# eigenkernel/eigenkernel

Measured on AMD Instinct MI355X. Metric: eigenpairs/s (full spectrum) + achieved fp64 TFLOP/s vs roofline, N=16384 GEP, higher is better.
Workload: dtype f64

## Files before the change

eigenkernel_amd/csrc/ek_common.h:

```cpp
#pragma once
#include <hip/hip_runtime.h>
#include <cstddef>
#include <cstdint>
#include <cstdio>

#define EK_HIP_CHECK(expr)                                                              \
  do {                                                                                  \
    hipError_t _e = (expr);                                                             \
    if (_e != hipSuccess) {                                                             \
      fprintf(stderr, "[ek_hip] %s failed at %s:%d: %s\n", #expr, __FILE__, __LINE__,   \
              hipGetErrorString(_e));                                                   \
      return -1000 - (int)_e;                                                           \
    }                                                                                   \
  } while (0)

namespace ek {

constexpr int kWave = 64;

inline int ceil_div(int a, int b) { return (a + b - 1) / b; }
inline int round_up(int a, int b) { return ceil_div(a, b) * b; }

struct GemmDesc {
  int M, N, K;
  bool transA, transB;
  double alpha, beta;
  const double *A; int lda; long long strideA;
  const double *B; int ldb; long long strideB;
  double *C; int ldc; long long strideC;
  int batch;
  bool lower_only;
  bool staged_rank_k = false;
  const long long *d_offs = nullptr;
  const int *d_dims = nullptr;
  bool even_offs = false;
  bool small_tiles = false;
};
void gemm(hipStream_t s, const GemmDesc &g);

enum { kGemmNone = -1, kGemmSmall = 0, kGemmW4 = 1, kGemmW8 = 2, kGemmRankK = 3 };
struct GemmPlan {
  int kernel;
  bool vec;
  int lower_only;
  int tile;
  int tiles_m, tiles_n;
  unsigned grid_x;
};
GemmPlan gemm_plan(const GemmDesc &g);
bool gemm_compact_tile(int tiles_m, int tiles_n, int tile, int &tm, int &tn);

inline void gemm(hipStream_t s, bool ta, bool tb, int M, int N, int K, double alpha,
                 const double *A, int lda, const double *B, int ldb, double beta, double *C,
                 int ldc, bool lower_only = false, bool staged_rank_k = false, bool small_tiles = false) {
  GemmDesc g{M, N, K, ta, tb, alpha, beta, A, lda, 0, B, ldb, 0, C, ldc, 0, 1, lower_only, staged_rank_k};
  g.small_tiles = small_tiles;
  gemm(s, g);
}

enum { kProfQ2Apply = 0, kProfChase = 1, kProfSymm = 2, kProfSyr2k = 3, kProfCount = 4 };
void kprof_enable(bool on);
bool kprof_enabled();
void kprof_begin(hipStream_t s, int id);
void kprof_end(hipStream_t s, int id);
void kprof_collect(double *seconds , long long *launches );

void copy_matrix(hipStream_t s, int m, int n, const double *src, int lds, double *dst, int ldd);
void set_matrix(hipStream_t s, int m, int n, double offdiag, double diag, double *A, int lda);
void symmetrize_lower(hipStream_t s, int n, double *A, int lda);
void transpose_rows(hipStream_t s, int n, int m, const double *src, int lds, int r0, double *dst, int ldd);
void gather_columns(hipStream_t s, int m, int n, const double *src, int lds, const int *perm,
                    double *dst, int ldd);

void gather_block_cyclic(hipStream_t s, int mr, int nc, const double *src, int lds, int nb, int pr,
                         int me_r, int pc, int me_c, double *dst, int ldd);

void scatter_block_cyclic(hipStream_t s, int mr, int nc, const double *src, int lds, int nb, int pr,
                          int me_r, int pc, int me_c, double *dst, int ldd);

void maxabs_lower(hipStream_t s, int n, const double *A, int lda, double *partial , int bw = 1 << 30);
void scale_lower(hipStream_t s, int n, double alpha, double *A, int lda);
void scale_vector(hipStream_t s, int n, double alpha, double *x);

// ... 140 lines not shown
```

eigenkernel_amd/csrc/ek_debug.hip:

```cpp
#include "ek_api_internal.h"

using namespace ek;
using namespace ek::api;

extern "C" {

int ek_hip_potrf_team(int n, double *B_loc, const int desc_B[9], int nteam, long long *mismatch) {
  if (n < 0) return -1;
  if (!B_loc && n > 0) return -2;
  int rc = check_desc(desc_B, 3, n, n); if (rc) return rc;
  if (nteam < 0 || nteam > kMaxTeam) return -4;
  rc = ensure_init(); if (rc) return rc;
  if (mismatch) *mismatch = 0;
  if (n == 0) return 0;
  std::lock_guard<std::mutex> lk(g_mu);
  if (nteam == 0 && !g_comm.on) return -4;
  hipStream_t s = g_ctx.stream;
  const int ld = pad_ld(n), nblk = ceil_div(n, kDiagNB);
  const int nmem = nteam > 0 ? nteam : 1, P = nteam > 0 ? nteam : g_comm.nranks;
  const size_t wb = potrf_dist_work_bytes(n, ld, P);
  const size_t per = al((size_t)ld * ld * 8) + al((size_t)nblk * kDiagNB * kDiagNB * 8) + al(wb) + 256;
  void *ws;
  rc = workspace(per * nmem + 256, &ws);
  if (rc) return rc;
// ... 695 lines not shown
  DevMem mem;
  if (offs && batch > 0) {
    double *p; rc = mem.alloc(&p, (size_t)3 * batch * sizeof(long long)); if (rc) return rc;
    EK_HIP_CHECK(hipMemcpy(p, offs, (size_t)3 * batch * sizeof(long long), hipMemcpyHostToDevice));
    g.d_offs = reinterpret_cast<const long long *>(p);
  }
  if (dims && batch > 0) {
    double *p; rc = mem.alloc(&p, (size_t)3 * batch * sizeof(int)); if (rc) return rc;
    EK_HIP_CHECK(hipMemcpy(p, dims, (size_t)3 * batch * sizeof(int), hipMemcpyHostToDevice));
    g.d_dims = reinterpret_cast<const int *>(p);
  }
  gemm_variant_out(gemm_plan(g), batch, variant);
  gemm(s, g);
  EK_HIP_CHECK(hipGetLastError());
  EK_HIP_CHECK(hipStreamSynchronize(s));
  return 0;
}

int ek_hip_debug_gemm_compact_map(int tiles_m, int tiles_n, long long first, int count, int *tm, int *tn, int *valid) {
  if (tiles_m < 1) return -1;
  if (tiles_n < 1 || tiles_n > tiles_m) return -2;
  if (first < 0) return -3;
  if (count < 0 || first + count > 0x7fffffffLL) return -4;
  if (count > 0 && (!tm || !tn)) return -5;
  int ok = 0;
  for (int i = 0; i < count; ++i) {
    const bool v = gemm_compact_tile(tiles_m, tiles_n, (int)(first + i), tm[i], tn[i]);
    if (valid) valid[i] = v ? 1 : 0;
    ok += v ? 1 : 0;
  }
  return ok;
}

int ek_hip_debug_sytrd_split(void *alt, int mask) {
  std::lock_guard<std::mutex> lk(g_mu);
  sytrd_debug_split(alt, mask);
  return 0;
}

int ek_hip_debug_set_sytrd_maxcols(int max_cols) {
  std::lock_guard<std::mutex> lk(g_mu);
  sytrd_set_max_cols(max_cols);
  return 0;
}

}
```

eigenkernel_amd/csrc/ek_gemm.hip:

```cpp
#include "ek_common.h"

#include <cmath>
#include <cstdlib>

namespace ek {
namespace {

typedef double double4_t __attribute__((ext_vector_type(4)));

constexpr int BM = 128, BN = 128, BK = 16;
constexpr int MC_LD = BM + 16;
constexpr int KC_LD = BK + 1;
constexpr int TILE_DOUBLES = (BK * MC_LD > BM * KC_LD) ? BK * MC_LD : BM * KC_LD;

struct GemmArgs {
  int M, N, K;
  double alpha, beta;
  const double *A; int lda; long long sA;
  const double *B; int ldb; long long sB;
  double *C; int ldc; long long sC;
  int lower_only;
  int tiles_m, tiles_n;
  const long long *offs;
  const int *dims;
};

template <bool KCONTIG>
__device__ __forceinline__ void load_slab(double (&r)[8], const double *__restrict__ P, int ld,
                                          int x0, int X, int k0, int K, int t) {
#pragma unroll
  for (int i = 0; i < 8; ++i) {
    const int idx = t + 256 * i;
    int x, k;
    if (KCONTIG) { k = idx & 15; x = idx >> 4; }
    else         { x = idx & 127; k = idx >> 7; }
    const int gx = x0 + x, gk = k0 + k;
    double v = 0.0;
    if (gx < X && gk < K)
      v = KCONTIG ? P[(size_t)gk + (size_t)gx * ld] : P[(size_t)gx + (size_t)gk * ld];
    r[i] = v;
  }
}

template <bool KCONTIG>
__device__ __forceinline__ void store_slab(const double (&r)[8], double *s, int t) {
// ... 8 lines not shown
typedef double double2g_t __attribute__((ext_vector_type(2)));
template <bool KCONTIG>
__device__ __forceinline__ void load_slab_v(double (&r)[8], const double *__restrict__ P, int ld, int x0, int X,
                                            int k0, int K, int t) {
  if (x0 + BM <= X && k0 + BK <= K) {
#pragma unroll
    for (int i = 0; i < 4; ++i) {
      const int idx = t + 256 * i;
      double2g_t v;
      if (KCONTIG) v = *reinterpret_cast<const double2g_t *>(P + (size_t)(k0 + 2 * (idx & 7)) + (size_t)(x0 + (idx >> 3)) * ld);
      else         v = *reinterpret_cast<const double2g_t *>(P + (size_t)(x0 + 2 * (idx & 63)) + (size_t)(k0 + (idx >> 6)) * ld);
      r[2 * i] = v.x; r[2 * i + 1] = v.y;
    }
  } else {
#pragma unroll
    for (int i = 0; i < 4; ++i) {
      const int idx = t + 256 * i;
#pragma unroll
      for (int h = 0; h < 2; ++h) {
        const int gx = x0 + (KCONTIG ? (idx >> 3) : 2 * (idx & 63) + h);
        const int gk = k0 + (KCONTIG ? 2 * (idx & 7) + h : (idx >> 6));
        double v = 0.0;
        if (gx < X && gk < K) v = KCONTIG ? P[(size_t)gk + (size_t)gx * ld] : P[(size_t)gx + (size_t)gk * ld];
        r[2 * i + h] = v;
      }
    }
  }
}
template <bool KCONTIG>
__device__ __forceinline__ void store_slab_v(const double (&r)[8], double *s, int t) {
#pragma unroll
  for (int i = 0; i < 4; ++i) {
    const int idx = t + 256 * i;
    if (KCONTIG) { const int k = 2 * (idx & 7), x = idx >> 3; s[x * KC_LD + k] = r[2 * i]; s[x * KC_LD + k + 1] = r[2 * i + 1]; }
    else { const int x = 2 * (idx & 63), k = idx >> 6; *reinterpret_cast<double2g_t *>(&s[k * MC_LD + x]) = (double2g_t){r[2 * i], r[2 * i + 1]}; }
  }
}

template <bool KCONTIG>
__device__ __forceinline__ double frag(const double *s, int x, int k) {
  return KCONTIG ? s[x * KC_LD + k] : s[k * MC_LD + x];
}

__host__ __device__ __forceinline__ bool tile_of(const GemmArgs &p, int tile, int &tm, int &tn) {
  if (p.lower_only == 2) {
    const long long T = p.tiles_m, c = tile;
    int j = (int)(((double)(2 * T + 1) - sqrt((double)((2 * T + 1) * (2 * T + 1) - 8 * c))) * 0.5);
    if (j < 0) j = 0;
    if (j > p.tiles_n - 1) j = p.tiles_n - 1;
    while (j + 1 < p.tiles_n && (long long)(j + 1) * T - (long long)(j + 1) * j / 2 <= c) ++j;
    while (j > 0 && (long long)j * T - (long long)j * (j - 1) / 2 > c) --j;
    tn = j; tm = j + (int)(c - ((long long)j * T - (long long)j * (j - 1) / 2));
    return tm < p.tiles_m;
  }
  tm = tile % p.tiles_m; tn = tile / p.tiles_m;
  return true;
}

template <bool TA, bool TB, bool VEC>
__global__ __launch_bounds__(256, 2) void gemm_kernel(GemmArgs p) {
  __shared__ __attribute__((aligned(16))) double smem[2 * TILE_DOUBLES];
  double *sA = smem, *sB = smem + TILE_DOUBLES;

  int tm, tn;
  if (!tile_of(p, blockIdx.x, tm, tn)) return;
  const int m0 = tm * BM, n0 = tn * BN;
  if (p.lower_only && n0 > m0 + BM - 1) return;
  if (p.dims) {
    p.M = p.dims[3 * blockIdx.y]; p.N = p.dims[3 * blockIdx.y + 1]; p.K = p.dims[3 * blockIdx.y + 2];
    if (m0 >= p.M || n0 >= p.N) return;
  }

  const double *__restrict__ A = p.A + (size_t)blockIdx.y * p.sA;
  const double *__restrict__ B = p.B + (size_t)blockIdx.y * p.sB;
  double *__restrict__ C = p.C + (size_t)blockIdx.y * p.sC;
  if (p.offs) {
    A += p.offs[3 * blockIdx.y]; B += p.offs[3 * blockIdx.y + 1]; C += p.offs[3 * blockIdx.y + 2];
  }

  const int t = threadIdx.x, lane = t & 63, wave = t >> 6;
  const int wm = (wave & 1) * 64, wn = (wave >> 1) * 64;
  const int l15 = lane & 15, l4 = lane >> 4;

  double4_t acc[4][4];
#pragma unroll
  for (int i = 0; i < 4; ++i)
#pragma unroll
    for (int j = 0; j < 4; ++j) acc[i][j] = (double4_t){0.0, 0.0, 0.0, 0.0};

  double ra[8], rb[8];
  if (VEC) {
    load_slab_v<TA>(ra, A, p.lda, m0, p.M, 0, p.K, t);
    load_slab_v<!TB>(rb, B, p.ldb, n0, p.N, 0, p.K, t);
  } else {
    load_slab<TA>(ra, A, p.lda, m0, p.M, 0, p.K, t);
    load_slab<!TB>(rb, B, p.ldb, n0, p.N, 0, p.K, t);
  }

  for (int k0 = 0; k0 < p.K; k0 += BK) {
    __syncthreads();
    if (VEC) { store_slab_v<TA>(ra, sA, t); store_slab_v<!TB>(rb, sB, t); }
    else { store_slab<TA>(ra, sA, t); store_slab<!TB>(rb, sB, t); }
    __syncthreads();
    if (k0 + BK < p.K) {
      if (VEC) {
        load_slab_v<TA>(ra, A, p.lda, m0, p.M, k0 + BK, p.K, t);
        load_slab_v<!TB>(rb, B, p.ldb, n0, p.N, k0 + BK, p.K, t);
      } else {
        load_slab<TA>(ra, A, p.lda, m0, p.M, k0 + BK, p.K, t);
        load_slab<!TB>(rb, B, p.ldb, n0, p.N, k0 + BK, p.K, t);
      }
    }
#pragma unroll
    for (int kk = 0; kk < BK; kk += 4) {
      double fa[4], fb[4];
#pragma unroll
      for (int i = 0; i < 4; ++i) {
        fa[i] = frag<TA>(sA, wm + i * 16 + l15, kk + l4);
        fb[i] = frag<!TB>(sB, wn + i * 16 + l15, kk + l4);
      }
#pragma unroll
      for (int ni = 0; ni < 4; ++ni)
#pragma unroll
        for (int mi = 0; mi < 4; ++mi)
          acc[ni][mi] = __builtin_amdgcn_mfma_f64_16x16x4f64(fb[ni], fa[mi], acc[ni][mi], 0, 0, 0);
    }
  }

  const double alpha = p.alpha, beta = p.beta;
#pragma unroll
  for (int ni = 0; ni < 4; ++ni)
#pragma unroll
    for (int mi = 0; mi < 4; ++mi) {
      const int m = m0 + wm + mi * 16 + l15;
#pragma unroll
      for (int r = 0; r < 4; ++r) {
        const int n = n0 + wn + ni * 16 + l4 + 4 * r;
        if (m < p.M && n < p.N) {
          double *c = C + (size_t)m + (size_t)n * p.ldc;
          double v = alpha * acc[ni][mi][r];
          if (beta != 0.0) v += beta * *c;
          *c = v;
        }
      }
    }
}


template <bool KCONTIG>
__device__ __forceinline__ void load_slab8(double (&r)[4], const double *__restrict__ P, int ld,
                                           int x0, int X, int k0, int K, int t) {
#pragma unroll
  for (int i = 0; i < 4; ++i) {
    const int idx = t + 512 * i;
    int x, k;
    if (KCONTIG) { k = idx & 15; x = idx >> 4; }
    else         { x = idx & 127; k = idx >> 7; }
    const int gx = x0 + x, gk = k0 + k;
    double v = 0.0;
// ... 14 lines not shown

template <bool KCONTIG>
__device__ __forceinline__ void load_slab8_v(double (&r)[4], const double *__restrict__ P, int ld, int x0, int X,
                                             int k0, int K, int t) {
  if (x0 + BM <= X && k0 + BK <= K) {
#pragma unroll
    for (int i = 0; i < 2; ++i) {
      const int idx = t + 512 * i;
      double2g_t v;
      if (KCONTIG) v = *reinterpret_cast<const double2g_t *>(P + (size_t)(k0 + 2 * (idx & 7)) + (size_t)(x0 + (idx >> 3)) * ld);
      else         v = *reinterpret_cast<const double2g_t *>(P + (size_t)(x0 + 2 * (idx & 63)) + (size_t)(k0 + (idx >> 6)) * ld);
      r[2 * i] = v.x; r[2 * i + 1] = v.y;
    }
  } else {
#pragma unroll
    for (int i = 0; i < 2; ++i) {
      const int idx = t + 512 * i;
#pragma unroll
      for (int h = 0; h < 2; ++h) {
        const int gx = x0 + (KCONTIG ? (idx >> 3) : 2 * (idx & 63) + h);
        const int gk = k0 + (KCONTIG ? 2 * (idx & 7) + h : (idx >> 6));
        double v = 0.0;
        if (gx < X && gk < K) v = KCONTIG ? P[(size_t)gk + (size_t)gx * ld] : P[(size_t)gx + (size_t)gk * ld];
        r[2 * i + h] = v;
      }
    }
  }
}
template <bool KCONTIG>
__device__ __forceinline__ void store_slab8_v(const double (&r)[4], double *s, int t) {
#pragma unroll
  for (int i = 0; i < 2; ++i) {
    const int idx = t + 512 * i;
    if (KCONTIG) { const int k = 2 * (idx & 7), x = idx >> 3; s[x * KC_LD + k] = r[2 * i]; s[x * KC_LD + k + 1] = r[2 * i + 1]; }
    else { const int x = 2 * (idx & 63), k = idx >> 6; *reinterpret_cast<double2g_t *>(&s[k * MC_LD + x]) = (double2g_t){r[2 * i], r[2 * i + 1]}; }
  }
}

template <bool TA, bool TB, bool VEC>
__global__ __launch_bounds__(512, 4) void gemm_kernel_w8(GemmArgs p) {
  __shared__ __attribute__((aligned(16))) double smem[2 * TILE_DOUBLES];
  double *sA = smem, *sB = smem + TILE_DOUBLES;
  int tm, tn;
  if (!tile_of(p, blockIdx.x, tm, tn)) return;
  const int m0 = tm * BM, n0 = tn * BN;
  if (p.lower_only && n0 > m0 + BM - 1) return;
  if (p.dims) {
    p.M = p.dims[3 * blockIdx.y]; p.N = p.dims[3 * blockIdx.y + 1]; p.K = p.dims[3 * blockIdx.y + 2];
    if (m0 >= p.M || n0 >= p.N) return;
  }
  const double *__restrict__ A = p.A + (size_t)blockIdx.y * p.sA;
  const double *__restrict__ B = p.B + (size_t)blockIdx.y * p.sB;
  double *__restrict__ C = p.C + (size_t)blockIdx.y * p.sC;
  if (p.offs) {
    A += p.offs[3 * blockIdx.y]; B += p.offs[3 * blockIdx.y + 1]; C += p.offs[3 * blockIdx.y + 2];
  }
  const int t = threadIdx.x, lane = t & 63, wave = t >> 6;
  const int wm = (wave & 1) * 64, wn = (wave >> 1) * 32;
  const int l15 = lane & 15, l4 = lane >> 4;
  double4_t acc[2][4];
#pragma unroll
  for (int i = 0; i < 2; ++i)
#pragma unroll
    for (int j = 0; j < 4; ++j) acc[i][j] = (double4_t){0.0, 0.0, 0.0, 0.0};
  double ra0[4], rb0[4];
  if (VEC) {
    load_slab8_v<TA>(ra0, A, p.lda, m0, p.M, 0, p.K, t);
    load_slab8_v<!TB>(rb0, B, p.ldb, n0, p.N, 0, p.K, t);
  } else {
    load_slab8<TA>(ra0, A, p.lda, m0, p.M, 0, p.K, t);
    load_slab8<!TB>(rb0, B, p.ldb, n0, p.N, 0, p.K, t);
  }
  for (int k0 = 0; k0 < p.K; k0 += BK) {
    __syncthreads();
    if (VEC) { store_slab8_v<TA>(ra0, sA, t); store_slab8_v<!TB>(rb0, sB, t); }
    else { store_slab8<TA>(ra0, sA, t); store_slab8<!TB>(rb0, sB, t); }
    __syncthreads();
// ... 160 lines not shown
      for (int ni = 0; ni < 2; ++ni)
#pragma unroll
        for (int mi = 0; mi < 2; ++mi)
          acc[ni][mi] = __builtin_amdgcn_mfma_f64_16x16x4f64(fb[ni], fa[mi], acc[ni][mi], 0, 0, 0);
    }
  }
  const double alpha = p.alpha, beta = p.beta;
#pragma unroll
  for (int ni = 0; ni < 2; ++ni)
#pragma unroll
    for (int mi = 0; mi < 2; ++mi) {
      const int m = m0 + wm + mi * 16 + l15;
#pragma unroll
      for (int r = 0; r < 4; ++r) {
        const int n = n0 + wn + ni * 16 + l4 + 4 * r;
        if (m < p.M && n < p.N) {
          double *c = C + (size_t)m + (size_t)n * p.ldc;
          double v = alpha * acc[ni][mi][r];
          if (beta != 0.0) v += beta * *c;
          *c = v;
        }
      }
    }
}

constexpr int RK = 32;
constexpr int RK_LD = BM + 16;
typedef double double2_t __attribute__((ext_vector_type(2)));

__global__ __launch_bounds__(512) void gemm_rankk_kernel(GemmArgs p) {
  extern __shared__ double rk_smem[];
  double *sA = rk_smem, *sB = rk_smem + RK * RK_LD;
  int tm, tn;
  if (!tile_of(p, blockIdx.x, tm, tn)) return;
  const int m0 = tm * BM, n0 = tn * BN;
  if (p.lower_only && n0 > m0 + BM - 1) return;
  if (p.dims) {
    p.M = p.dims[3 * blockIdx.y]; p.N = p.dims[3 * blockIdx.y + 1]; p.K = p.dims[3 * blockIdx.y + 2];
    if (m0 >= p.M || n0 >= p.N) return;
  }
  const double *__restrict__ A = p.A + (size_t)blockIdx.y * p.sA;
  const double *__restrict__ B = p.B + (size_t)blockIdx.y * p.sB;
  double *__restrict__ C = p.C + (size_t)blockIdx.y * p.sC;
  if (p.offs) { A += p.offs[3 * blockIdx.y]; B += p.offs[3 * blockIdx.y + 1]; C += p.offs[3 * blockIdx.y + 2]; }
  const int t = threadIdx.x, lane = t & 63, wave = t >> 6;
  const int wm = (wave & 1) * 64, wn = (wave >> 1) * 32;
  const int l15 = lane & 15, l4 = lane >> 4;
  const bool vec = ((p.lda | p.ldb) & 1) == 0 && ((((size_t)A | (size_t)B) & 15) == 0);
  const int xp = 2 * (t & 63), kq = t >> 6;
  constexpr int NF = RK / 8;
  double2_t ra[NF], rb[NF];
  auto fetch = [&](int k0) {
#pragma unroll
    for (int i = 0; i < NF; ++i) {
      const int k = k0 + kq + 8 * i;
      double2_t va = (double2_t){0.0, 0.0}, vb = (double2_t){0.0, 0.0};
      if (k < p.K) {
        const double *pa = A + (size_t)(m0 + xp) + (size_t)k * p.lda;
        const double *pb = B + (size_t)(n0 + xp) + (size_t)k * p.ldb;
        if (vec && m0 + xp + 1 < p.M) va = *reinterpret_cast<const double2_t *>(pa);
        else { if (m0 + xp < p.M) va.x = pa[0]; if (m0 + xp + 1 < p.M) va.y = pa[1]; }
        if (vec && n0 + xp + 1 < p.N) vb = *reinterpret_cast<const double2_t *>(pb);
        else { if (n0 + xp < p.N) vb.x = pb[0]; if (n0 + xp + 1 < p.N) vb.y = pb[1]; }
      }
      ra[i] = va; rb[i] = vb;
    }
  };
// ... 63 lines not shown
    }
}

}

GemmPlan gemm_plan(const GemmDesc &g) {
  GemmPlan pl;
  pl.kernel = kGemmNone; pl.vec = false; pl.lower_only = 0; pl.tile = 0; pl.tiles_m = pl.tiles_n = 0; pl.grid_x = 0;
  if (g.M <= 0 || g.N <= 0 || g.batch <= 0) return pl;
  pl.lower_only = g.lower_only ? 1 : 0;
  const long long big_tiles = (long long)ceil_div(g.M, BM) * ceil_div(g.N, BN) * g.batch;
  const bool compact = g.lower_only && g.batch == 1 && !g.d_dims && !g.d_offs;
  static int vec_env = -1;
  if (vec_env < 0) { const char *e = getenv("EK_GEMM_VEC"); vec_env = e ? atoi(e) : 1; }
  pl.vec = vec_env && (!g.d_offs || g.even_offs) && ((g.lda | g.ldb) & 1) == 0 &&
           ((((size_t)g.A | (size_t)g.B) & 15) == 0) && (g.batch == 1 || ((g.strideA | g.strideB) & 1) == 0);
  const bool small = (big_tiles < 256 && !g.lower_only) || (g.lower_only && g.small_tiles);
  pl.tile = small ? SM : BM;
  pl.tiles_m = ceil_div(g.M, pl.tile); pl.tiles_n = ceil_div(g.N, pl.tile);
  pl.grid_x = (unsigned)(pl.tiles_m * pl.tiles_n);
  if (compact && pl.tiles_n <= pl.tiles_m) {
    pl.lower_only = 2;
    pl.grid_x = (unsigned)((long long)pl.tiles_n * pl.tiles_m - (long long)pl.tiles_n * (pl.tiles_n - 1) / 2);
  }
  if (small) { pl.kernel = kGemmSmall; return pl; }
  static int w8 = -2;
  if (w8 == -2) { const char *e = getenv("EK_GEMM_W8"); w8 = e ? atoi(e) : -1; }
  static int rankk = -1;
  if (rankk < 0) { const char *e = getenv("EK_GEMM_RANKK"); rankk = e ? atoi(e) : 1; }
  if (rankk && g.staged_rank_k && !g.transA && g.transB && g.K <= 256 && g.K >= 32 && w8 < 0) { pl.kernel = kGemmRankK; return pl; }
  const bool use_w8 = (w8 >= 0) ? (w8 != 0) : (g.K <= 512 && g.beta != 0.0);
  pl.kernel = use_w8 ? kGemmW8 : kGemmW4;
  return pl;
}

bool gemm_compact_tile(int tiles_m, int tiles_n, int tile, int &tm, int &tn) {
  GemmArgs p;
  p.lower_only = 2; p.tiles_m = tiles_m; p.tiles_n = tiles_n;
  return tile_of(p, tile, tm, tn);
}

void gemm(hipStream_t s, const GemmDesc &g) {
  const GemmPlan pl = gemm_plan(g);
  if (pl.kernel == kGemmNone) return;
  GemmArgs p;
  p.M = g.M; p.N = g.N; p.K = g.K > 0 ? g.K : 0;
  p.alpha = g.alpha; p.beta = g.beta;
  p.A = g.A; p.lda = g.lda; p.sA = g.strideA;
  p.B = g.B; p.ldb = g.ldb; p.sB = g.strideB;
  p.C = g.C; p.ldc = g.ldc; p.sC = g.strideC;
  p.lower_only = pl.lower_only;
  p.offs = g.d_offs; p.dims = g.d_dims;
  p.tiles_m = pl.tiles_m; p.tiles_n = pl.tiles_n;
  const bool vec = pl.vec;
  if (pl.kernel == kGemmSmall) {
    dim3 sgrid(pl.grid_x, g.batch), sblock(256);
    if (vec) {
      if (!g.transA && !g.transB) hipLaunchKernelGGL((gemm_small_kernel<false, false, true>), sgrid, sblock, 0, s, p);
      else if (!g.transA && g.transB) hipLaunchKernelGGL((gemm_small_kernel<false, true, true>), sgrid, sblock, 0, s, p);
      else if (g.transA && !g.transB) hipLaunchKernelGGL((gemm_small_kernel<true, false, true>), sgrid, sblock, 0, s, p);
      else hipLaunchKernelGGL((gemm_small_kernel<true, true, true>), sgrid, sblock, 0, s, p);
      return;
    }
    if (!g.transA && !g.transB) hipLaunchKernelGGL((gemm_small_kernel<false, false, false>), sgrid, sblock, 0, s, p);
    else if (!g.transA && g.transB) hipLaunchKernelGGL((gemm_small_kernel<false, true, false>), sgrid, sblock, 0, s, p);
    else if (g.transA && !g.transB) hipLaunchKernelGGL((gemm_small_kernel<true, false, false>), sgrid, sblock, 0, s, p);
    else hipLaunchKernelGGL((gemm_small_kernel<true, true, false>), sgrid, sblock, 0, s, p);
    return;
  }
  dim3 grid(pl.grid_x, g.batch), block(256);
  static bool rk_attr = false;
  if (!rk_attr) {
    rk_attr = true;
    (void)hipFuncSetAttribute((const void *)gemm_rankk_kernel, hipFuncAttributeMaxDynamicSharedMemorySize,
                              2 * RK * RK_LD * (int)sizeof(double));
  }
  if (pl.kernel == kGemmRankK) {
    hipLaunchKernelGGL(gemm_rankk_kernel, grid, dim3(512), 2 * RK * RK_LD * sizeof(double), s, p);
    return;
  }
  if (pl.kernel == kGemmW8) {
    dim3 b8(512);
    if (vec) {
      if (!g.transA && !g.transB) hipLaunchKernelGGL((gemm_kernel_w8<false, false, true>), grid, b8, 0, s, p);
      else if (!g.transA && g.transB) hipLaunchKernelGGL((gemm_kernel_w8<false, true, true>), grid, b8, 0, s, p);
      else if (g.transA && !g.transB) hipLaunchKernelGGL((gemm_kernel_w8<true, false, true>), grid, b8, 0, s, p);
      else hipLaunchKernelGGL((gemm_kernel_w8<true, true, true>), grid, b8, 0, s, p);
      return;
    }
    if (!g.transA && !g.transB) hipLaunchKernelGGL((gemm_kernel_w8<false, false, false>), grid, b8, 0, s, p);
    else if (!g.transA && g.transB) hipLaunchKernelGGL((gemm_kernel_w8<false, true, false>), grid, b8, 0, s, p);
    else if (g.transA && !g.transB) hipLaunchKernelGGL((gemm_kernel_w8<true, false, false>), grid, b8, 0, s, p);
    else hipLaunchKernelGGL((gemm_kernel_w8<true, true, false>), grid, b8, 0, s, p);
    return;
  }
  if (vec) {
    if (!g.transA && !g.transB) hipLaunchKernelGGL((gemm_kernel<false, false, true>), grid, block, 0, s, p);
    else if (!g.transA && g.transB) hipLaunchKernelGGL((gemm_kernel<false, true, true>), grid, block, 0, s, p);
    else if (g.transA && !g.transB) hipLaunchKernelGGL((gemm_kernel<true, false, true>), grid, block, 0, s, p);
    else hipLaunchKernelGGL((gemm_kernel<true, true, true>), grid, block, 0, s, p);
    return;
  }
  if (!g.transA && !g.transB) hipLaunchKernelGGL((gemm_kernel<false, false, false>), grid, block, 0, s, p);
  else if (!g.transA && g.transB) hipLaunchKernelGGL((gemm_kernel<false, true, false>), grid, block, 0, s, p);
  else if (g.transA && !g.transB) hipLaunchKernelGGL((gemm_kernel<true, false, false>), grid, block, 0, s, p);
  else hipLaunchKernelGGL((gemm_kernel<true, true, false>), grid, block, 0, s, p);
}

}
```

eigenkernel_amd/solver.py:

```python
import ctypes
import os
from dataclasses import dataclass, field

import numpy as np

from . import descriptor as _d

_HERE = os.path.dirname(os.path.abspath(__file__))
LIB_PATH = os.environ.get("EK_HIP_LIB") or os.path.join(_HERE, "csrc", "libek_hip.so")

N_STAGES = 8
SOLVERS = ("hip", "hip_select", "general_hip", "general_hip_select")
REPLACES = {"hip": "scalapack", "hip_select": "scalapack_select",
            "general_hip": "general_scalapack", "general_hip_select": "general_scalapack_select"}


class LibraryMissing(RuntimeError):
    pass


_lib = None
_dp = ctypes.POINTER(ctypes.c_double)
_ip = ctypes.POINTER(ctypes.c_int)
_llp = ctypes.POINTER(ctypes.c_longlong)
# ... 41 lines not shown
        "ek_hip_comm_size": (c_int, []),
        "ek_hip_comm_rank": (c_int, []),
        "ek_hip_comm_destroy": (c_int, []),
        "ek_hip_comm_allreduce_device": (c_int, [vp, ctypes.c_longlong]),
        "ek_hip_stedc": (c_int, [c_int, _dp, _dp, _dp, _ip]),
        "ek_hip_ormtr": (c_int, [c_int, c_int, _dp, _ip, _dp, _dp, _ip]),
        "ek_hip_trtrs": (c_int, [c_int, c_int, _dp, _ip, _dp, _ip]),
        "ek_hip_dgemm": (c_int, [c_int, c_int, c_int, c_int, c_int, c_dbl, _dp, c_int, _dp, c_int,
                                 c_dbl, _dp, c_int, c_int]),
        "ek_hip_malloc": (c_int, [ctypes.POINTER(vp), c_ull]),
        "ek_hip_free": (c_int, [vp]),
        "ek_hip_memcpy_h2d": (c_int, [vp, vp, c_ull]),
        "ek_hip_memcpy_d2h": (c_int, [vp, vp, c_ull]),
        "ek_hip_synchronize": (c_int, []),
        "ek_hip_synth_matrix_device": (c_int, [c_int, c_ull, vp, c_int]),
        "ek_hip_residual_device": (c_int, [c_int, c_int, c_int, vp, c_int, vp, c_int, vp, vp, c_int, _dp, _dp, _dp]),
        "ek_hip_orthogonality_device": (c_int, [c_int, c_int, c_int, c_int, vp, c_int, vp, c_int, _dp]),
        "ek_hip_ipratios_device": (c_int, [c_int, c_int, c_int, vp, c_int, vp, c_int, _dp]),
        "ek_hip_check": (c_int, [c_int, c_int, c_int, c_int, c_int, c_int, _dp, _ip, _dp, _ip, _dp, _dp, _ip, _dp]),
        "ek_hip_profile_symv": (c_int, [c_int]),
        "ek_hip_debug_sytrd": (c_int, [c_int, c_int, c_int, _dp]),
        "ek_hip_debug_sytrd_team": (c_int, [c_int, c_int, c_int, _dp]),
        "ek_hip_debug_set_sytrd_maxcols": (c_int, [c_int]),
        "ek_hip_debug_sytrd_work_bytes": (ctypes.c_ulonglong, [c_int]),
        "ek_hip_debug_sytrd_split": (c_int, [vp, c_int]),
        "ek_hip_debug_gemm_at": (c_int, [c_int, c_int, c_int, c_int, c_int, vp, c_int, vp, c_int, c_dbl, vp, c_int,
                                         c_int, c_int, _dp]),
        "ek_hip_debug_sytrd_at": (c_int, [c_int, c_int, c_int, vp, vp, vp, _dp]),
        "ek_hip_debug_gemm_desc": (c_int, [c_int] * 5 + [c_dbl, c_dbl, vp, c_int, c_ll, vp, c_int, c_ll, vp, c_int, c_ll]
                                   + [c_int] * 5 + [_llp, _ip, _ip]),
        "ek_hip_debug_gemm_plan": (c_int, [c_int] * 5 + [c_dbl, c_dbl, vp, c_int, c_ll, vp, c_int, c_ll, vp, c_int, c_ll]
                                   + [c_int] * 5 + [_llp, _ip, _ip]),
        "ek_hip_debug_gemm_compact_map": (c_int, [c_int, c_int, c_ll, c_int, _ip, _ip, _ip]),
        "ek_hip_debug_reduce_team": (c_int, [c_int, c_int, c_int, _dp]),
        "ek_hip_profile_symv_get": (c_int, [_dp, ctypes.POINTER(ctypes.c_longlong), _dp]),
        "ek_hip_debug_sy2sb": (c_int, [c_int, _dp, c_int, _dp, c_int, _dp, _ip]),
        "ek_hip_debug_sb2st": (c_int, [c_int, _dp, c_int, _dp, _dp, _dp, c_int, c_int, _ip]),
        "ek_hip_debug_two_stage_timing": (c_int, [c_int, c_int, c_int, _dp, _ip]),
        "ek_hip_debug_set_two_stage": (c_int, [c_int]),
        "ek_hip_profile_kernels": (c_int, [c_int]),
        "ek_hip_profile_kernels_get": (c_int, [_dp, _llp]),
        "ek_hip_debug_last_solve_stats": (c_int, [_dp, c_int]),
        "ek_hip_debug_sy2sb_team": (c_int, [c_int, _dp, c_int, _dp, c_int, _dp, c_int, _ip, _llp]),
        "ek_hip_debug_sy2sb_team_timing": (c_int, [c_int, c_int, c_int, _dp]),
        "ek_hip_debug_sy2sb_team_profile": (c_int, [c_int, c_int, c_int, c_int, _dp, _dp]),
        "ek_hip_debug_fail_next_chase": (c_int, [c_int]),
        "ek_hip_debug_stedc_team": (c_int, [c_int, c_int, c_int]),
        "ek_hip_debug_potrf_team_profile": (c_int, [c_int, c_int]),
        "ek_hip_debug_potrf_team_profile_get": (c_int, [c_int, _dp]),
        "ek_hip_debug_stedc_team_get": (c_int, [_dp]),
        "ek_hip_debug_last_pipe_stats": (c_int, [_dp, c_int]),
        "ek_hip_debug_workspace_bytes": (ctypes.c_ulonglong, [c_int, c_int, c_int, c_int, ctypes.POINTER(ctypes.c_ulonglong)]),
        "ek_hip_eigenvalues_device": (c_int, [c_int, c_int, c_int, c_int, vp, c_int, vp, c_int, vp, _dp, c_int]),
        "ek_hip_eigenvalues": (c_int, [c_int, c_int, c_int, c_int, _dp, c_int, _dp, c_int, _dp, _dp, c_int]),
        "ek_hip_stebz": (c_int, [c_int, _dp, _dp, c_int, c_int, _dp]),
        "ek_hip_debug_values_workspace_bytes": (ctypes.c_ulonglong, [c_int, c_int]),
        "ek_hip_debug_set_stebz": (c_int, [c_int]),
        "ek_hip_eigenpairs_device": (c_int, [c_int, c_int, c_int, c_int, c_dbl, c_dbl, c_int, c_int, vp, c_int, vp, c_int,
                                             _ip, _ip, vp, vp, c_int, c_int, _dp, c_int]),
        "ek_hip_eigenpairs": (c_int, [c_int, c_int, c_int, c_int, c_dbl, c_dbl, c_int, c_int, _dp, c_int, _dp, c_int,
                                      _ip, _ip, _dp, _dp, c_int, c_int, _dp, c_int]),
        "ek_hip_stebz_range": (c_int, [c_int, _dp, _dp, c_dbl, c_dbl, _ip, _ip, _dp]),
        "ek_hip_debug_window_workspace_bytes": (ctypes.c_ulonglong, [c_int, c_int, c_int, c_int, c_int]),
        "ek_hip_sygvx_device": (c_int, [c_int, c_int, c_int, c_int, c_dbl, c_dbl, c_int, c_int, vp, c_int, vp, c_int,
                                        _ip, _ip, vp, vp, c_int, c_int, _dp, c_int]),
        "ek_hip_sygvx": (c_int, [c_int, c_int, c_int, c_int, c_dbl, c_dbl, c_int, c_int, _dp, c_int, _dp, c_int,
# ... 19 lines not shown
        "ek_hip_check_batched": (c_int, [c_int, c_int, c_int, _dp, c_int, c_ll, _dp, c_int, c_ll, _dp, _dp, c_int, c_ll,
                                         _ip, _dp, _dp, _dp]),
        "ek_hip_check_vbatched_device": (c_int, [c_int, c_int, _ip, vp, _ip, vp, _ip, vp, vp, _ip, _ip, _dp, vp, _dp]),
        "ek_hip_check_vbatched": (c_int, [c_int, c_int, _ip, vp, _ip, vp, _ip, vp, vp, _ip, _ip, _dp, vp, _dp]),
        "ek_hip_debug_vbatched_streams": (c_int, [c_int]),
        "ek_hip_debug_vbatched_last": (c_int, [_dp, _ip]),
    }
    for name, (res, args) in sigs.items():
        try:
            fn = getattr(lib, name)
        except AttributeError:
            if os.environ.get("EK_HIP_BRINGUP") == "1":
                continue
            raise
        fn.restype = res
        fn.argtypes = args
    if path is None:
        _lib = lib
    return lib


EXPORTED_SYMBOLS = (
    "ek_hip_version", "ek_hip_init", "ek_hip_finalize", "ek_hip_stage_name", "ek_hip_solve",
    "ek_hip_solve_device", "ek_hip_solve_replicated", "ek_hip_solve_device_grid",
    "ek_hip_set_allgatherv", "ek_hip_gather_matrix", "ek_hip_potrf", "ek_hip_sygst", "ek_hip_sytrd", "ek_hip_stedc",
    "ek_hip_ormtr", "ek_hip_trtrs", "ek_hip_dgemm", "ek_hip_malloc", "ek_hip_free",
    "ek_hip_memcpy_h2d", "ek_hip_memcpy_d2h", "ek_hip_synchronize", "ek_hip_synth_matrix_device",
    "ek_hip_profile_symv", "ek_hip_profile_symv_get", "ek_hip_debug_sytrd",
    "ek_hip_residual_device", "ek_hip_orthogonality_device", "ek_hip_ipratios_device", "ek_hip_check",
    "ek_hip_sytrd_team", "ek_hip_comm_unique_id", "ek_hip_comm_init", "ek_hip_comm_size", "ek_hip_comm_rank",
    "ek_hip_comm_destroy", "ek_hip_comm_allreduce_device", "ek_hip_debug_sytrd_team", "ek_hip_sygst_team",
    "ek_hip_potrf_team", "ek_hip_debug_reduce_team", "ek_hip_comm_attach_host",
    "ek_hip_debug_set_sytrd_maxcols", "ek_hip_debug_sytrd_work_bytes", "ek_hip_debug_sytrd_at", "ek_hip_debug_sytrd_split", "ek_hip_debug_gemm_at",
    "ek_hip_debug_gemm_desc", "ek_hip_debug_gemm_plan", "ek_hip_debug_gemm_compact_map",
    "ek_hip_debug_sy2sb", "ek_hip_debug_sb2st", "ek_hip_debug_two_stage_timing", "ek_hip_debug_set_two_stage",
    "ek_hip_profile_kernels", "ek_hip_profile_kernels_get", "ek_hip_debug_last_solve_stats",
    "ek_hip_debug_sy2sb_team", "ek_hip_debug_sy2sb_team_timing", "ek_hip_debug_sy2sb_team_profile", "ek_hip_debug_workspace_bytes", "ek_hip_debug_fail_next_chase", "ek_hip_debug_last_pipe_stats",
    "ek_hip_debug_stedc_team", "ek_hip_debug_stedc_team_get",
    "ek_hip_debug_potrf_team_profile", "ek_hip_debug_potrf_team_profile_get",
    "ek_hip_eigenvalues_device", "ek_hip_eigenvalues", "ek_hip_stebz",
    "ek_hip_debug_values_workspace_bytes", "ek_hip_debug_set_stebz",
    "ek_hip_eigenpairs_device", "ek_hip_eigenpairs", "ek_hip_stebz_range", "ek_hip_debug_window_workspace_bytes",
    "ek_hip_sygvx_device", "ek_hip_sygvx", "ek_hip_sygst_ibtype", "ek_hip_trmm", "ek_hip_debug_sygvx_workspace_bytes",
    "ek_hip_eigenpairs_batched_device", "ek_hip_eigenpairs_batched",
    "ek_hip_eigenpairs_vbatched_device", "ek_hip_eigenpairs_vbatched",
    "ek_hip_debug_vbatched_streams", "ek_hip_debug_vbatched_last",
    "ek_hip_check_batched_device", "ek_hip_check_batched", "ek_hip_check_vbatched_device", "ek_hip_check_vbatched",
    "ek_hip_sygv_batched_device", "ek_hip_sygv_batched", "ek_hip_sygv_vbatched_device", "ek_hip_sygv_vbatched",
)


def _check(what, A, B, w, Z, n_cols, index1=1, index2=1):
    lib = load_library()
    Z = _farr(Z)
    n = Z.shape[0]
    A_ = _farr(A) if A is not None else None
    B_ = _farr(B) if B is not None else None
    out = np.zeros(max(3, n))
    wv = np.ascontiguousarray(np.asarray(w, dtype=np.float64)) if w is not None else np.zeros(max(n, 1))
    info = lib.ek_hip_check(what, 1 if B is not None else 0, n, n_cols, index1, index2,
                            _P(A_) if A_ is not None else None, _I(_desc_for(A_)) if A_ is not None else None,
                            _P(B_) if B_ is not None else None, _I(_desc_for(B_)) if B_ is not None else None,
                            _P(wv), _P(Z), _I(_desc_for(Z)), _P(out))
    if info:
        raise RuntimeError("ek_hip_check(%d) info=%d" % (what, info))
    return out

# ... 726 lines not shown
```

include/ek_hip_debug.h:

```cpp
#ifndef EK_HIP_DEBUG_H
#define EK_HIP_DEBUG_H

#ifdef __cplusplus
extern "C" {
#endif

int ek_hip_profile_symv(int enable);
int ek_hip_profile_symv_get(double *seconds, long long *launches, double *algorithmic_bytes);

int ek_hip_profile_kernels(int enable);
int ek_hip_profile_kernels_get(double *seconds , long long *launches );

int ek_hip_debug_sytrd(int n, int ld, int reps, double *seconds);
unsigned long long ek_hip_debug_sytrd_work_bytes(int n);
int ek_hip_debug_sytrd_at(int n, int max_cols, int reps, double *dA, void *work, double *vecs, double *seconds);
int ek_hip_debug_gemm_at(int transa, int transb, int m, int n, int k, const double *dA, int lda, const double *dB,
                         int ldb, double beta, double *dC, int ldc, int lower_only, int reps, double *seconds);
int ek_hip_debug_gemm_desc(int transa, int transb, int m, int n, int k, double alpha, double beta, const double *dA, int lda,
                           long long strideA, const double *dB, int ldb, long long strideB, double *dC, int ldc,
                           long long strideC, int batch, int lower_only, int staged_rank_k, int small_tiles, int even_offs,
                           const long long *offs, const int *dims, int *variant );
int ek_hip_debug_gemm_plan(int transa, int transb, int m, int n, int k, double alpha, double beta, const double *dA, int lda,
                           long long strideA, const double *dB, int ldb, long long strideB, double *dC, int ldc,
                           long long strideC, int batch, int lower_only, int staged_rank_k, int small_tiles, int even_offs,
                           const long long *offs, const int *dims, int *variant );
int ek_hip_debug_gemm_compact_map(int tiles_m, int tiles_n, long long first, int count, int *tm, int *tn, int *valid);
int ek_hip_debug_sytrd_split(void *alt, int mask);
int ek_hip_debug_set_sytrd_maxcols(int max_cols);
int ek_hip_debug_sytrd_team(int n, int nteam, int reps, double *seconds);
int ek_hip_debug_reduce_team(int n, int nteam, int reps, double *seconds );

int ek_hip_debug_sy2sb(int n, double *A, int lda, double *V, int ldv, double *tau, int *flag);
int ek_hip_debug_sb2st(int n, const double *A, int lda, double *d, double *e, double *Z, int ldz, int ncols, int *flag);
int ek_hip_debug_two_stage_timing(int n, int ncols, int reps, double *seconds, int *flag);
int ek_hip_debug_set_two_stage(int min_order);
int ek_hip_debug_sy2sb_team(int n, double *A, int lda, double *V, int ldv, double *tau, int nteam, int *flag,
                            long long *mismatch);
int ek_hip_debug_sy2sb_team_timing(int n, int nteam, int reps, double *seconds);
int ek_hip_debug_sy2sb_team_profile(int n, int nteam, int reps, int lookahead_min, double *seconds, double *parts);

int ek_hip_debug_last_solve_stats(double *out, int count);

unsigned long long ek_hip_debug_workspace_bytes(int problem, int n, int n_vec, int nranks, unsigned long long *parts);

unsigned long long ek_hip_debug_values_workspace_bytes(int problem, int n);
int ek_hip_debug_set_stebz(int lanes);
unsigned long long ek_hip_debug_window_workspace_bytes(int problem, int n, int jobz, int range, int m);
unsigned long long ek_hip_debug_sygvx_workspace_bytes(int itype, int n, int jobz, int range, int m);
int ek_hip_debug_vbatched_streams(int streams);
int ek_hip_debug_vbatched_last(double *class_seconds, int *class_count);

int ek_hip_debug_fail_next_chase(int times);

int ek_hip_debug_stedc_team(int nranks, int levels, int profile);
int ek_hip_debug_stedc_team_get(double *seconds);

int ek_hip_debug_potrf_team_profile(int lookahead, int profile);
int ek_hip_debug_potrf_team_profile_get(int nteam, double *parts);

// ... 7 lines not shown
```

Baseline: 20190.

## Double-buffer W4 GEMM LDS, add XCD-aware tile swizzle, pad K-contig stride

The W4 GEMM kernel moves to dynamic shared memory with two LDS stages, so the next slab is stored while the current one is multiplied, dropping one barrier per K step. Block indices are remapped by a tile permutation that spreads consecutive blocks across 8 groups (matching the MI355X XCD count) and walks 8-row bands, aiming for better L2 locality, and it handles the compact lower-triangular grid too. KC_LD is padded to an even stride so K-contiguous slabs can be written as double2 vector stores. The costs are double the LDS per block, which can reduce occupancy, extra index arithmetic per block, and a debug entry point for the ordering.

```diff
diff --git a/eigenkernel_amd/csrc/ek_common.h b/eigenkernel_amd/csrc/ek_common.h
--- a/eigenkernel_amd/csrc/ek_common.h
+++ b/eigenkernel_amd/csrc/ek_common.h
@@ -49,6 +49,7 @@
 };
 GemmPlan gemm_plan(const GemmDesc &g);
 bool gemm_compact_tile(int tiles_m, int tiles_n, int tile, int &tm, int &tn);
+int gemm_tile_order(int b, int grid_x, int tiles_m, int tiles_n, bool compact);
 
 inline void gemm(hipStream_t s, bool ta, bool tb, int M, int N, int K, double alpha,
                  const double *A, int lda, const double *B, int ldb, double beta, double *C,
diff --git a/eigenkernel_amd/csrc/ek_debug.hip b/eigenkernel_amd/csrc/ek_debug.hip
--- a/eigenkernel_amd/csrc/ek_debug.hip
+++ b/eigenkernel_amd/csrc/ek_debug.hip
@@ -751,6 +751,20 @@
   return ok;
 }
 
+int ek_hip_debug_gemm_order(int tiles_m, int tiles_n, int compact, long long first, int count, int *index) {
+  if (tiles_m < 1) return -1;
+  if (tiles_n < 1 || (compact && tiles_n > tiles_m)) return -2;
+  if (compact != 0 && compact != 1) return -3;
+  const long long grid = compact ? (long long)tiles_n * tiles_m - (long long)tiles_n * (tiles_n - 1) / 2
+                                 : (long long)tiles_m * tiles_n;
+  if (grid > 0x7fffffffLL) return -1;
+  if (first < 0) return -4;
+  if (count < 0 || first + count > grid) return -5;
+  if (count > 0 && !index) return -6;
+  for (int i = 0; i < count; ++i) index[i] = gemm_tile_order((int)(first + i), (int)grid, tiles_m, tiles_n, compact != 0);
+  return count;
+}
+
 int ek_hip_debug_sytrd_split(void *alt, int mask) {
   std::lock_guard<std::mutex> lk(g_mu);
   sytrd_debug_split(alt, mask);
diff --git a/eigenkernel_amd/csrc/ek_gemm.hip b/eigenkernel_amd/csrc/ek_gemm.hip
--- a/eigenkernel_amd/csrc/ek_gemm.hip
+++ b/eigenkernel_amd/csrc/ek_gemm.hip
@@ -10,7 +10,7 @@
 
 constexpr int BM = 128, BN = 128, BK = 16;
 constexpr int MC_LD = BM + 16;
-constexpr int KC_LD = BK + 1;
+constexpr int KC_LD = BK + 2;
 constexpr int TILE_DOUBLES = (BK * MC_LD > BM * KC_LD) ? BK * MC_LD : BM * KC_LD;
 
 struct GemmArgs {
@@ -85,8 +85,8 @@
 #pragma unroll
   for (int i = 0; i < 4; ++i) {
     const int idx = t + 256 * i;
-    if (KCONTIG) { const int k = 2 * (idx & 7), x = idx >> 3; s[x * KC_LD + k] = r[2 * i]; s[x * KC_LD + k + 1] = r[2 * i + 1]; }
-    else { const int x = 2 * (idx & 63), k = idx >> 6; *reinterpret_cast<double2g_t *>(&s[k * MC_LD + x]) = (double2g_t){r[2 * i], r[2 * i + 1]}; }
+    const int o = KCONTIG ? (idx >> 3) * KC_LD + 2 * (idx & 7) : (idx >> 6) * MC_LD + 2 * (idx & 63);
+    *reinterpret_cast<double2g_t *>(&s[o]) = (double2g_t){r[2 * i], r[2 * i + 1]};
   }
 }
 
@@ -110,13 +110,44 @@
   return true;
 }
 
+__host__ __device__ __forceinline__ int tile_perm(int b, int grid_x, int tiles_m, int tiles_n, int lower_only) {
+  const int per = grid_x >> 3, rem = grid_x & 7, r = b & 7;
+  const long long q = (long long)r * per + (r < rem ? r : rem) + (b >> 3);
+  if (lower_only != 2) {
+    const long long band = q / (8LL * tiles_n);
+    const int r0 = 8 * (int)band, h = tiles_m - r0 < 8 ? tiles_m - r0 : 8;
+    const int qb = (int)(q - band * 8LL * tiles_n);
+    return (r0 + qb % h) + (qb / h) * tiles_m;
+  }
+  const long long N = tiles_n, tri = N * (N + 1) / 2;
+  auto S = [&](long long R) { return R <= N ? R * (R + 1) / 2 : tri + (R - N) * N; };
+  long long R = q < tri ? (long long)((sqrt((double)(8 * q + 1)) - 1.0) * 0.5) : N + (q - tri) / N;
+  if (R < 0) R = 0;
+  if (R > tiles_m - 1) R = tiles_m - 1;
+  while (R + 1 < tiles_m && S(R + 1) <= q) ++R;
+  while (R > 0 && S(R) > q) --R;
+  const int r0 = 8 * (int)(R >> 3), h = tiles_m - r0 < 8 ? tiles_m - r0 : 8;
+  int qb = (int)(q - S(r0));
+  const int full = r0 + 1 < tiles_n ? r0 + 1 : tiles_n;
+  int tm, tn;
+  if (qb < full * h) { tn = qb / h; tm = r0 + qb % h; }
+  else {
+    qb -= full * h;
+    int d = 1;
+    while (d < h - 1 && qb >= h - d) { qb -= h - d; ++d; }
+    tn = r0 + d; tm = tn + qb;
+  }
+  return (int)((long long)tn * tiles_m - (long long)tn * (tn - 1) / 2 + (tm - tn));
+}
+
+constexpr int W4_LDS_BYTES = 4 * TILE_DOUBLES * (int)sizeof(double);
+
 template <bool TA, bool TB, bool VEC>
 __global__ __launch_bounds__(256, 2) void gemm_kernel(GemmArgs p) {
-  __shared__ __attribute__((aligned(16))) double smem[2 * TILE_DOUBLES];
-  double *sA = smem, *sB = smem + TILE_DOUBLES;
+  extern __shared__ __attribute__((aligned(16))) double w4_smem[];
 
   int tm, tn;
-  if (!tile_of(p, blockIdx.x, tm, tn)) return;
+  if (!tile_of(p, tile_perm(blockIdx.x, gridDim.x, p.tiles_m, p.tiles_n, p.lower_only), tm, tn)) return;
   const int m0 = tm * BM, n0 = tn * BN;
   if (p.lower_only && n0 > m0 + BM - 1) return;
   if (p.dims) {
@@ -142,28 +173,22 @@
     for (int j = 0; j < 4; ++j) acc[i][j] = (double4_t){0.0, 0.0, 0.0, 0.0};
 
   double ra[8], rb[8];
-  if (VEC) {
-    load_slab_v<TA>(ra, A, p.lda, m0, p.M, 0, p.K, t);
-    load_slab_v<!TB>(rb, B, p.ldb, n0, p.N, 0, p.K, t);
-  } else {
-    load_slab<TA>(ra, A, p.lda, m0, p.M, 0, p.K, t);
-    load_slab<!TB>(rb, B, p.ldb, n0, p.N, 0, p.K, t);
-  }
-
-  for (int k0 = 0; k0 < p.K; k0 += BK) {
-    __syncthreads();
+  auto load = [&](int k0) {
+    if (VEC) {
+      load_slab_v<TA>(ra, A, p.lda, m0, p.M, k0, p.K, t);
+      load_slab_v<!TB>(rb, B, p.ldb, n0, p.N, k0, p.K, t);
+    } else {
+      load_slab<TA>(ra, A, p.lda, m0, p.M, k0, p.K, t);
+      load_slab<!TB>(rb, B, p.ldb, n0, p.N, k0, p.K, t);
+    }
+  };
+  auto store = [&](double *sA) {
+    double *sB = sA + TILE_DOUBLES;
     if (VEC) { store_slab_v<TA>(ra, sA, t); store_slab_v<!TB>(rb, sB, t); }
     else { store_slab<TA>(ra, sA, t); store_slab<!TB>(rb, sB, t); }
-    __syncthreads();
-    if (k0 + BK < p.K) {
-      if (VEC) {
-        load_slab_v<TA>(ra, A, p.lda, m0, p.M, k0 + BK, p.K, t);
-        load_slab_v<!TB>(rb, B, p.ldb, n0, p.N, k0 + BK, p.K, t);
-      } else {
-        load_slab<TA>(ra, A, p.lda, m0, p.M, k0 + BK, p.K, t);
-        load_slab<!TB>(rb, B, p.ldb, n0, p.N, k0 + BK, p.K, t);
-      }
-    }
+  };
+  auto multiply = [&](const double *sA) {
+    const double *sB = sA + TILE_DOUBLES;
 #pragma unroll
     for (int kk = 0; kk < BK; kk += 4) {
       double fa[4], fb[4];
@@ -178,6 +203,23 @@
         for (int mi = 0; mi < 4; ++mi)
           acc[ni][mi] = __builtin_amdgcn_mfma_f64_16x16x4f64(fb[ni], fa[mi], acc[ni][mi], 0, 0, 0);
     }
+  };
+
+  load(0);
+  store(w4_smem);
+  if (BK < p.K) load(BK);
+  __syncthreads();
+  auto step = [&](int k0, double *cur, double *nxt) {
+    if (k0 + BK < p.K) {
+      store(nxt);
+      if (k0 + 2 * BK < p.K) load(k0 + 2 * BK);
+    }
+    multiply(cur);
+    __syncthreads();
+  };
+  for (int k0 = 0; k0 < p.K; k0 += 2 * BK) {
+    step(k0, w4_smem, w4_smem + 2 * TILE_DOUBLES);
+    if (k0 + BK < p.K) step(k0 + BK, w4_smem + 2 * TILE_DOUBLES, w4_smem);
   }
 
   const double alpha = p.alpha, beta = p.beta;
@@ -258,8 +300,8 @@
 #pragma unroll
   for (int i = 0; i < 2; ++i) {
     const int idx = t + 512 * i;
-    if (KCONTIG) { const int k = 2 * (idx & 7), x = idx >> 3; s[x * KC_LD + k] = r[2 * i]; s[x * KC_LD + k + 1] = r[2 * i + 1]; }
-    else { const int x = 2 * (idx & 63), k = idx >> 6; *reinterpret_cast<double2g_t *>(&s[k * MC_LD + x]) = (double2g_t){r[2 * i], r[2 * i + 1]}; }
+    const int o = KCONTIG ? (idx >> 3) * KC_LD + 2 * (idx & 7) : (idx >> 6) * MC_LD + 2 * (idx & 63);
+    *reinterpret_cast<double2g_t *>(&s[o]) = (double2g_t){r[2 * i], r[2 * i + 1]};
   }
 }
 
@@ -268,7 +310,7 @@
   __shared__ __attribute__((aligned(16))) double smem[2 * TILE_DOUBLES];
   double *sA = smem, *sB = smem + TILE_DOUBLES;
   int tm, tn;
-  if (!tile_of(p, blockIdx.x, tm, tn)) return;
+  if (!tile_of(p, tile_perm(blockIdx.x, gridDim.x, p.tiles_m, p.tiles_n, p.lower_only), tm, tn)) return;
   const int m0 = tm * BM, n0 = tn * BN;
   if (p.lower_only && n0 > m0 + BM - 1) return;
   if (p.dims) {
@@ -495,7 +537,7 @@
   extern __shared__ double rk_smem[];
   double *sA = rk_smem, *sB = rk_smem + RK * RK_LD;
   int tm, tn;
-  if (!tile_of(p, blockIdx.x, tm, tn)) return;
+  if (!tile_of(p, tile_perm(blockIdx.x, gridDim.x, p.tiles_m, p.tiles_n, p.lower_only), tm, tn)) return;
   const int m0 = tm * BM, n0 = tn * BN;
   if (p.lower_only && n0 > m0 + BM - 1) return;
   if (p.dims) {
@@ -625,6 +667,10 @@
   const bool use_w8 = (w8 >= 0) ? (w8 != 0) : (g.K <= 512 && g.beta != 0.0);
   pl.kernel = use_w8 ? kGemmW8 : kGemmW4;
   return pl;
+}
+
+int gemm_tile_order(int b, int grid_x, int tiles_m, int tiles_n, bool compact) {
+  return tile_perm(b, grid_x, tiles_m, tiles_n, compact ? 2 : 0);
 }
 
 bool gemm_compact_tile(int tiles_m, int tiles_n, int tile, int &tm, int &tn) {
@@ -667,6 +713,11 @@
     rk_attr = true;
     (void)hipFuncSetAttribute((const void *)gemm_rankk_kernel, hipFuncAttributeMaxDynamicSharedMemorySize,
                               2 * RK * RK_LD * (int)sizeof(double));
+    const void *w4[8] = {(const void *)gemm_kernel<false, false, true>, (const void *)gemm_kernel<false, true, true>,
+                         (const void *)gemm_kernel<true, false, true>, (const void *)gemm_kernel<true, true, true>,
+                         (const void *)gemm_kernel<false, false, false>, (const void *)gemm_kernel<false, true, false>,
+                         (const void *)gemm_kernel<true, false, false>, (const void *)gemm_kernel<true, true, false>};
+    for (const void *f : w4) (void)hipFuncSetAttribute(f, hipFuncAttributeMaxDynamicSharedMemorySize, W4_LDS_BYTES);
   }
   if (pl.kernel == kGemmRankK) {
     hipLaunchKernelGGL(gemm_rankk_kernel, grid, dim3(512), 2 * RK * RK_LD * sizeof(double), s, p);
@@ -688,16 +739,16 @@
     return;
   }
   if (vec) {
-    if (!g.transA && !g.transB) hipLaunchKernelGGL((gemm_kernel<false, false, true>), grid, block, 0, s, p);
-    else if (!g.transA && g.transB) hipLaunchKernelGGL((gemm_kernel<false, true, true>), grid, block, 0, s, p);
-    else if (g.transA && !g.transB) hipLaunchKernelGGL((gemm_kernel<true, false, true>), grid, block, 0, s, p);
-    else hipLaunchKernelGGL((gemm_kernel<true, true, true>), grid, block, 0, s, p);
+    if (!g.transA && !g.transB) hipLaunchKernelGGL((gemm_kernel<false, false, true>), grid, block, W4_LDS_BYTES, s, p);
+    else if (!g.transA && g.transB) hipLaunchKernelGGL((gemm_kernel<false, true, true>), grid, block, W4_LDS_BYTES, s, p);
+    else if (g.transA && !g.transB) hipLaunchKernelGGL((gemm_kernel<true, false, true>), grid, block, W4_LDS_BYTES, s, p);
+    else hipLaunchKernelGGL((gemm_kernel<true, true, true>), grid, block, W4_LDS_BYTES, s, p);
     return;
   }
-  if (!g.transA && !g.transB) hipLaunchKernelGGL((gemm_kernel<false, false, false>), grid, block, 0, s, p);
-  else if (!g.transA && g.transB) hipLaunchKernelGGL((gemm_kernel<false, true, false>), grid, block, 0, s, p);
-  else if (g.transA && !g.transB) hipLaunchKernelGGL((gemm_kernel<true, false, false>), grid, block, 0, s, p);
-  else hipLaunchKernelGGL((gemm_kernel<true, true, false>), grid, block, 0, s, p);
-}
-
-}
+  if (!g.transA && !g.transB) hipLaunchKernelGGL((gemm_kernel<false, false, false>), grid, block, W4_LDS_BYTES, s, p);
+  else if (!g.transA && g.transB) hipLaunchKernelGGL((gemm_kernel<false, true, false>), grid, block, W4_LDS_BYTES, s, p);
+  else if (g.transA && !g.transB) hipLaunchKernelGGL((gemm_kernel<true, false, false>), grid, block, W4_LDS_BYTES, s, p);
+  else hipLaunchKernelGGL((gemm_kernel<true, true, false>), grid, block, W4_LDS_BYTES, s, p);
+}
+
+}
diff --git a/eigenkernel_amd/solver.py b/eigenkernel_amd/solver.py
--- a/eigenkernel_amd/solver.py
+++ b/eigenkernel_amd/solver.py
@@ -97,6 +97,7 @@
         "ek_hip_debug_gemm_plan": (c_int, [c_int] * 5 + [c_dbl, c_dbl, vp, c_int, c_ll, vp, c_int, c_ll, vp, c_int, c_ll]
                                    + [c_int] * 5 + [_llp, _ip, _ip]),
         "ek_hip_debug_gemm_compact_map": (c_int, [c_int, c_int, c_ll, c_int, _ip, _ip, _ip]),
+        "ek_hip_debug_gemm_order": (c_int, [c_int, c_int, c_int, c_ll, c_int, _ip]),
         "ek_hip_debug_reduce_team": (c_int, [c_int, c_int, c_int, _dp]),
         "ek_hip_profile_symv_get": (c_int, [_dp, ctypes.POINTER(ctypes.c_longlong), _dp]),
         "ek_hip_debug_sy2sb": (c_int, [c_int, _dp, c_int, _dp, c_int, _dp, _ip]),
@@ -182,7 +183,7 @@
     "ek_hip_comm_destroy", "ek_hip_comm_allreduce_device", "ek_hip_debug_sytrd_team", "ek_hip_sygst_team",
     "ek_hip_potrf_team", "ek_hip_debug_reduce_team", "ek_hip_comm_attach_host",
     "ek_hip_debug_set_sytrd_maxcols", "ek_hip_debug_sytrd_work_bytes", "ek_hip_debug_sytrd_at", "ek_hip_debug_sytrd_split", "ek_hip_debug_gemm_at",
-    "ek_hip_debug_gemm_desc", "ek_hip_debug_gemm_plan", "ek_hip_debug_gemm_compact_map",
+    "ek_hip_debug_gemm_desc", "ek_hip_debug_gemm_plan", "ek_hip_debug_gemm_compact_map", "ek_hip_debug_gemm_order",
     "ek_hip_debug_sy2sb", "ek_hip_debug_sb2st", "ek_hip_debug_two_stage_timing", "ek_hip_debug_set_two_stage",
     "ek_hip_profile_kernels", "ek_hip_profile_kernels_get", "ek_hip_debug_last_solve_stats",
     "ek_hip_debug_sy2sb_team", "ek_hip_debug_sy2sb_team_timing", "ek_hip_debug_sy2sb_team_profile", "ek_hip_debug_workspace_bytes", "ek_hip_debug_fail_next_chase", "ek_hip_debug_last_pipe_stats",
diff --git a/include/ek_hip_debug.h b/include/ek_hip_debug.h
--- a/include/ek_hip_debug.h
+++ b/include/ek_hip_debug.h
@@ -25,6 +25,7 @@
                            long long strideC, int batch, int lower_only, int staged_rank_k, int small_tiles, int even_offs,
                            const long long *offs, const int *dims, int *variant );
 int ek_hip_debug_gemm_compact_map(int tiles_m, int tiles_n, long long first, int count, int *tm, int *tn, int *valid);
+int ek_hip_debug_gemm_order(int tiles_m, int tiles_n, int compact, long long first, int count, int *index);
 int ek_hip_debug_sytrd_split(void *alt, int mask);
 int ek_hip_debug_set_sytrd_maxcols(int max_cols);
 int ek_hip_debug_sytrd_team(int n, int nteam, int reps, double *seconds);
```

Result: no change. 20170 (-0.1%).
